# zhengjingsen/LidarDetection

Hardware: AMD Instinct MI355X
Metric: frames/sec (fwd+NMS) PointPillar-KITTI (higher is better)
Workload: dtype f32; 1 GPU; PointPillar-KITTI bs=16 per GPU, fp32, eval BN folded: HIP voxelize + PFN; dense 2D backbone = first layer from the pillars (sparse implicit GEMM), stride-1 3x3 layers as Winograd F(4x4,3x3) on the fp32 MFMA, strided deblocks as one fused MFMA GEMM (all this repo's HIP), the two stride-2 3x3 layers MIOpen, stride-1 deblock + 1x1 heads hipBLASLt; exact HIP top-k + decode + batched rotated NMS; clou; replicas=1

## Files before the change

### include/lidar_hip.h

```cpp
#ifndef LIDAR_HIP_H
#define LIDAR_HIP_H

#include <stddef.h>
#include <stdint.h>

#ifdef __cplusplus
extern "C" {
#endif

#define LIDAR_OK 0
#define LIDAR_ERR_ARG (-1)
#define LIDAR_ERR_LAUNCH (-2)
#define LIDAR_ERR_WORKSPACE (-3)
#define LIDAR_ERR_UNSUPPORTED (-4)

size_t lidar_voxelize_workspace_bytes(int batch, int n_max, int max_voxels);
int lidar_voxelize_workspace_init(void *ws, size_t ws_bytes, int batch, int n_max, int max_voxels, void *stream);
int lidar_voxelize(const float *points, const int *point_offsets, int batch, int n_max, int num_features,
                   const float *range6, const float *voxel_size3, const int *grid3, int max_points,
                   int max_voxels, int compact, int algo, float *voxels, int *coords, int *num_points,
                   int *voxel_offsets, void *ws, size_t ws_bytes, void *stream);
int lidar_voxelize_hostoff(const float *points, const int *point_offsets, const int *host_offsets, int batch, int n_max,
                           int num_features, const float *range6, const float *voxel_size3, const int *grid3, int max_points,
                           int max_voxels, int compact, int algo, float *voxels, int *coords, int *num_points,
// ... 192 lines not shown
                                             int n_out, int K, int Cin, int Cout, const float *packed, const float *bias,
                                             const float *residual, int relu, float *out_features, void *stream);
int lidar_spconv_wgrad(const float *in_features, const float *grad_out, const int *nbr, int n_out, int K, int Cin, int Cout,
                       float *grad_weight, void *stream);
int lidar_spconv_wgrad_mfma_supported(int K, int Cin, int Cout);
size_t lidar_spconv_wgrad_workspace_bytes(int n_out, int K, int Cin, int Cout);
int lidar_spconv_wgrad_mfma(const float *in_features, const float *grad_out, const int *nbr, const int *order, int n_out, int K,
                            int Cin, int Cout, float *grad_weight, void *ws, size_t ws_bytes, void *stream);
size_t lidar_sparse_to_dense_workspace_bytes(int batch, int D, int H, int W);
int lidar_sparse_to_dense(const float *features, const int *indices, int n, int channels, int batch, int D, int H, int W,
                          float *out, void *ws, size_t ws_bytes, void *stream);

int lidar_bias_act_nhwc(const float *in, const float *bias, long long n_pix, int C, int relu, float *out, int out_C,
                        int out_off, void *stream);
int lidar_bias_act_upsample_nhwc(const float *in, const float *bias, int batch, int h, int w, int s, int C, int relu,
                                 float *out, int out_C, int out_off, void *stream);
int lidar_dense_gemm_bias_act(const float *A, long long M, int K, const float *W, int N, const float *bias, int relu,
                              float *D, int ldd, void *ws, size_t ws_bytes, void *stream);
int lidar_dense_gemm_export_choices(int *out7, int cap);
int lidar_dense_gemm_import_choices(const int *in7, int n);

size_t lidar_wino_packed_floats(int Cin, int Cout);
int lidar_wino_supported(int Cin, int Cout);
int lidar_wino_pack_weights(const float *w, int Cin, int Cout, float *packed, void *stream);
int lidar_wino_conv3x3_nhwc(const float *in, int B, int H, int W, int Cin, const float *packed, const float *bias, int relu, int Cout,
                            float *out, int out_C, int out_off, void *stream);
int lidar_wino_conv3x3_grouped_nhwc(const float *in, int B, int H, int W, int in_C, int group_cin, int n_groups, const float *packed,
                                    const float *bias, int relu, float *out, int out_C, int out_off, void *stream);
int lidar_wino_conv3x3_grouped_compact_nhwc(const float *in, int B, int H, int W, int in_C, int group_cin, int n_groups,
                                            const float *packed, const float *bias, int relu, const int *grp_cout, const int *grp_ooff,
                                            float *out, int out_C, int out_off, void *stream);

size_t lidar_wino43_packed_floats(int Cin, int Cout);
int lidar_wino43_supported(int Cin, int Cout);
int lidar_wino43_pack_weights(const float *w, int Cin, int Cout, float *packed, void *stream);
int lidar_wino43_conv3x3_nhwc(const float *in, int B, int H, int W, int Cin, int in_C, const float *packed, const float *bias, int relu,
                              int Cout, float *out, int out_C, int out_off, void *stream);
size_t lidar_wino43s_packed_floats(int Cin, int Cout);
int lidar_wino43s_supported(int Cin, int Cout);
int lidar_wino43s_pack_weights(const float *w, int Cin, int Cout, float *packed, void *stream);
int lidar_wino43s_conv3x3_nhwc(const float *in, int B, int H, int W, int Cin, int in_C, const float *packed, const float *bias, int relu,
                               int Cout, float *out, int out_C, int out_off, void *stream);

int lidar_wino43_wgrad_supported(int Cin, int Cout);
size_t lidar_wino43_wgrad_workspace_bytes(int B, int H, int W, int Cin, int Cout);
int lidar_wino43_wgrad_nhwc(const float *x, int x_ld, const float *g, int g_ld, int B, int H, int W, int Cin, int Cout, float *dw,
                            void *ws, size_t ws_bytes, void *stream);

size_t lidar_deconv_packed_floats(int K, int N);
int lidar_deconv_supported(int K, int s, int C_up);
int lidar_deconv_pack_weights(const float *W, int K, int N, float *packed, void *stream);
int lidar_deconv_gemm_nhwc(const float *in, int B, int h, int w, int K, const float *packed, const float *bias, int relu, int s, int C_up,
                           float *out, int out_C, int out_off, void *stream);

#define LIDAR_DECONV_TRAIN_MIN_K 16
#define LIDAR_DECONV_TRAIN_MIN_CUP 32
#define LIDAR_DECONV_TRAIN_MAX_C 512
int lidar_deconv_train_supported(int K, int s, int C_up);
size_t lidar_deconv_wgrad_workspace_bytes(int B, int h, int w, int K, int s, int C_up);
int lidar_deconv_dgrad_nhwc(const float *g, int g_ld, const float *W, int B, int h, int w, int K, int s, int C_up, float *dx, int dx_ld,
                            void *stream);
int lidar_deconv_wgrad_nhwc(const float *x, int x_ld, const float *g, int g_ld, int B, int h, int w, int K, int s, int C_up, float *dw,
                            void *ws, size_t ws_bytes, void *stream);

int lidar_anchor_scores(const float *head, long long n_loc, int row_stride, int cls_off, int anchors_per_loc, int num_class,
                        float score_thresh, float *scores, unsigned char *labels, void *stream);
int lidar_decode_topk(const float *head, int batch, long long locs_per_frame, int row_stride, int box_off, int dir_off,
                      int anchors_per_loc, int num_dir_bins, const long long *top_idx, int k, const float *anchors,
                      float dir_offset, float dir_limit_offset, float period, float *boxes, void *stream);
size_t lidar_topk_workspace_bytes(int batch, long long n);
int lidar_topk_workspace_init(void *ws, size_t ws_bytes, int batch, long long n, void *stream);
int lidar_anchor_scores_hist(const float *head, int batch, long long locs_per_frame, int row_stride, int cls_off, int anchors_per_loc,
                             int num_class, float score_thresh, float *scores, unsigned char *labels, void *ws, size_t ws_bytes,
                             void *stream);
int lidar_topk_desc(const float *scores, int batch, long long n, int k, float valid_min, float score_max, int hist_ready,
                    float *top_scores, long long *top_idx, int *counts, void *ws, size_t ws_bytes, void *stream);
int lidar_post_nms_gather(const float *boxes, const float *top_scores, const long long *top_idx, const unsigned char *labels,
                          const long long *keep, const int *num_keep, int batch, int k, long long n, int keep_stride, int post,
                          float *out_boxes, float *out_scores, long long *out_labels, int *out_num, void *stream);

size_t lidar_anchor_assign_workspace_bytes(int batch, int max_gt, int num_classes);
int lidar_anchor_assign(const float *const *anchors, const long long *counts, const long long *per_loc, const long long *out_off,
                        const float *matched, const float *unmatched, const int *remap, int num_classes, int anchor_dim,
                        long long a_total, const signed char *class_of_id, const float *gt, const float *gt_enlarged, int batch,
                        int max_gt, int gt_cols, int code_size, int sincos, int norm_by_num_examples, int *labels, float *targets,
                        float *weights, void *ws, size_t ws_bytes, void *stream);

int lidar_atss_assign_supported(const long long *counts, int num_sets, int anchor_dim, int gt_cols, int code_size, int sincos,
                                int topk, int max_gt, int match_height);
size_t lidar_atss_assign_workspace_bytes(int batch, int max_gt, int num_sets, int topk);
int lidar_atss_assign(const float *const *anchors, const long long *counts, int num_sets, int anchor_dim, const float *gt, int batch,
                      int max_gt, int gt_cols, int code_size, int sincos, int topk, int match_height, int *labels, float *targets,
                      float *weights, void *ws, size_t ws_bytes, void *stream);

#define LIDAR_PROPOSAL_TARGET_MAX_ROIS 1024
#define LIDAR_PROPOSAL_TARGET_MAX_GT 512
#define LIDAR_PROPOSAL_TARGET_MAX_SAMPLES 512
#define LIDAR_PROPOSAL_TARGET_MAX_DIM 16
int lidar_proposal_target_supported(int num_rois, int max_gt, int roi_per_image, int box_dim);
int lidar_proposal_target(const float *rois, const float *roi_scores, const long long *roi_labels, const float *gt_boxes,
                          const float *gt_boxes_enlarged, int batch, int num_rois, int max_gt, int box_dim, int roi_per_image,
                          int fg_rois_per_image, const int *hard_quota, int by_class, int cls_score_type, float reg_fg_thresh,
                          float cls_fg_thresh, float cls_bg_thresh, float cls_bg_thresh_lo, float cls_fg_minus_bg,
                          const float *fg_keys, const float *draws, float *out_rois, float *out_gt_of_rois,
                          float *out_gt_of_rois_src, float *out_iou, float *out_scores, long long *out_labels,
                          long long *out_reg_valid, float *out_cls_labels, int *out_sampled, int *frame_status,
// ... 112 lines not shown
```

### lidardetection_amd/_lib.py

```python
import ctypes as C
import os

_HERE = os.path.dirname(os.path.abspath(__file__))
SO_PATH = os.environ.get("LIDAR_HIP_SO") or os.path.join(_HERE, "csrc", "liblidar_hip.so")

vp, i32, f32, sz = C.c_void_p, C.c_int, C.c_float, C.c_size_t

SIGNATURES = {
    "lidar_voxelize_workspace_bytes": (sz, [i32, i32, i32]),
    "lidar_voxelize_workspace_init": (i32, [vp, sz, i32, i32, i32, vp]),
    "lidar_voxelize": (i32, [vp, vp, i32, i32, i32, vp, vp, vp, i32, i32, i32, i32, vp, vp, vp, vp, vp, sz, vp]),
    "lidar_voxelize_hostoff": (i32, [vp, vp, vp, i32, i32, i32, vp, vp, vp, i32, i32, i32, i32, vp, vp, vp, vp, vp, sz, vp]),
    "lidar_voxelize_error_flag": (i32, [vp, sz, i32, i32, i32]),
    "lidar_timer_create": (vp, []),
    "lidar_timer_destroy": (None, [vp]),
    "lidar_voxelize_time_next": (None, [vp]),
    "lidar_timer_elapsed_ms": (C.c_float, [vp]),
    "lidar_timer_parts_ms": (i32, [vp, vp]),
    "lidar_voxelize_set_error_mirror": (i32, [vp, sz, i32, i32, i32, vp, vp]),
    "lidar_pillar_vfe": (i32, [vp, vp, vp, i32, vp, i32, i32, vp, vp, vp, i32, vp, vp, i32, i32, i32, vp, vp]),
    "lidar_mean_vfe": (i32, [vp, vp, i32, i32, i32, i32, vp, vp]),
    "lidar_pillar_scatter_workspace_bytes": (sz, [i32, i32, i32]),
    "lidar_pillar_scatter": (i32, [vp, vp, i32, i32, vp, i32, i32, i32, i32, i32, vp, vp, sz, vp]),
    "lidar_pillar_scatter_update": (i32, [vp, vp, i32, i32, vp, i32, i32, i32, i32, vp, vp, vp, vp]),
# ... 59 lines not shown
    "lidar_spconv_grid_init": (i32, [vp, sz, vp]),
    "lidar_spconv_grid_rows": (i32, [vp, i32, vp, i32, i32, i32, i32, vp, i32, vp]),
    "lidar_spconv_grid_table": (i32, [vp, i32, i32, i32, i32, i32, i32, i32, i32, i32, i32, i32, i32, i32, i32, vp, i32, vp, vp]),
    "lidar_spconv_grid_table_t": (i32, [vp, i32, i32, i32, i32, i32, i32, i32, i32, i32, i32, i32, i32, i32, i32, vp, i32, vp, vp]),
    "lidar_spconv_grid_pad_rows": (i32, [vp, vp, i32, vp]),
    "lidar_spconv_transpose_table": (i32, [vp, i32, i32, i32, vp, vp]),
    "lidar_spconv_grid_outputs_workspace_bytes": (sz, [i32, i32]),
    "lidar_spconv_grid_outputs": (i32, [vp, i32, i32, i32, i32, i32, i32, i32, i32, i32, i32, i32, i32, i32, i32, vp, vp, vp, vp, sz, vp]),
    "lidar_spconv_implicit_gemm": (i32, [vp, vp, i32, i32, i32, i32, vp, vp, vp, vp]),
    "lidar_spconv_implicit_gemm_fused": (i32, [vp, vp, i32, i32, i32, i32, vp, vp, vp, i32, vp, vp]),
    "lidar_spconv_row_masks": (i32, [vp, i32, i32, vp, vp]),
    "lidar_spconv_mask_group_workspace_bytes": (sz, [i32]),
    "lidar_spconv_mask_group_init": (i32, [vp, sz, vp]),
    "lidar_spconv_mask_group": (i32, [vp, i32, i32, vp, vp, vp, sz, vp]),
    "lidar_spconv_sorted_gemm_supported": (i32, [i32, i32, i32]),
    "lidar_spconv_implicit_gemm_sorted": (i32, [vp, vp, vp, vp, i32, i32, i32, i32, vp, vp, vp, i32, vp, vp]),
    "lidar_spconv_packed_floats": (sz, [i32, i32, i32]),
    "lidar_spconv_pack_weights": (i32, [vp, i32, i32, i32, vp, vp]),
    "lidar_spconv_implicit_gemm_sorted_packed": (i32, [vp, vp, vp, vp, i32, i32, i32, i32, vp, vp, vp, i32, vp, vp]),
    "lidar_spconv_wgrad": (i32, [vp, vp, vp, i32, i32, i32, i32, vp, vp]),
    "lidar_spconv_wgrad_mfma_supported": (i32, [i32, i32, i32]),
    "lidar_spconv_wgrad_workspace_bytes": (sz, [i32, i32, i32, i32]),
    "lidar_spconv_wgrad_mfma": (i32, [vp, vp, vp, vp, i32, i32, i32, i32, vp, vp, sz, vp]),
    "lidar_sparse_to_dense_workspace_bytes": (sz, [i32, i32, i32, i32]),
    "lidar_sparse_to_dense": (i32, [vp, vp, i32, i32, i32, i32, i32, i32, vp, vp, sz, vp]),
    "lidar_sparse_to_bev_nhwc": (i32, [vp, vp, i32, i32, i32, i32, i32, i32, vp, vp, sz, vp]),
    "lidar_sparse_to_bev_nhwc_backward": (i32, [vp, i32, i32, vp, i32, i32, i32, i32, i32, i32, vp, vp]),
    "lidar_bias_act_nhwc": (i32, [vp, vp, C.c_longlong, i32, i32, vp, i32, i32, vp]),
    "lidar_bias_act_upsample_nhwc": (i32, [vp, vp, i32, i32, i32, i32, i32, i32, vp, i32, i32, vp]),
    "lidar_dense_gemm_bias_act": (i32, [vp, C.c_longlong, i32, vp, i32, vp, i32, vp, i32, vp, sz, vp]),
    "lidar_dense_gemm_export_choices": (i32, [vp, i32]),
    "lidar_dense_gemm_import_choices": (i32, [vp, i32]),
    "lidar_wino_packed_floats": (sz, [i32, i32]),
    "lidar_wino_supported": (i32, [i32, i32]),
    "lidar_wino_pack_weights": (i32, [vp, i32, i32, vp, vp]),
    "lidar_wino_conv3x3_nhwc": (i32, [vp, i32, i32, i32, i32, vp, vp, i32, i32, vp, i32, i32, vp]),
    "lidar_wino43_packed_floats": (sz, [i32, i32]),
    "lidar_wino43_supported": (i32, [i32, i32]),
    "lidar_wino43_pack_weights": (i32, [vp, i32, i32, vp, vp]),
    "lidar_wino43_conv3x3_nhwc": (i32, [vp, i32, i32, i32, i32, i32, vp, vp, i32, i32, vp, i32, i32, vp]),
    "lidar_wino43s_packed_floats": (sz, [i32, i32]),
    "lidar_wino43s_supported": (i32, [i32, i32]),
    "lidar_wino43s_pack_weights": (i32, [vp, i32, i32, vp, vp]),
    "lidar_wino43s_conv3x3_nhwc": (i32, [vp, i32, i32, i32, i32, i32, vp, vp, i32, i32, vp, i32, i32, vp]),
    "lidar_wino43_wgrad_supported": (i32, [i32, i32]),
    "lidar_wino43_wgrad_workspace_bytes": (sz, [i32, i32, i32, i32, i32]),
    "lidar_wino43_wgrad_nhwc": (i32, [vp, i32, vp, i32, i32, i32, i32, i32, i32, vp, vp, sz, vp]),
    "lidar_wino_conv3x3_grouped_nhwc": (i32, [vp, i32, i32, i32, i32, i32, i32, vp, vp, i32, vp, i32, i32, vp]),
    "lidar_wino_conv3x3_grouped_compact_nhwc": (i32, [vp, i32, i32, i32, i32, i32, i32, vp, vp, i32, vp, vp, vp, i32, i32, vp]),
    "lidar_deconv_packed_floats": (sz, [i32, i32]),
    "lidar_deconv_supported": (i32, [i32, i32, i32]),
    "lidar_deconv_pack_weights": (i32, [vp, i32, i32, vp, vp]),
    "lidar_deconv_gemm_nhwc": (i32, [vp, i32, i32, i32, i32, vp, vp, i32, i32, i32, vp, i32, i32, vp]),
    "lidar_deconv_train_supported": (i32, [i32, i32, i32]),
    "lidar_deconv_wgrad_workspace_bytes": (sz, [i32, i32, i32, i32, i32, i32]),
    "lidar_deconv_dgrad_nhwc": (i32, [vp, i32, vp, i32, i32, i32, i32, i32, i32, vp, i32, vp]),
    "lidar_deconv_wgrad_nhwc": (i32, [vp, i32, vp, i32, i32, i32, i32, i32, i32, i32, vp, vp, sz, vp]),
    "lidar_anchor_scores": (i32, [vp, C.c_longlong, i32, i32, i32, i32, f32, vp, vp, vp]),
    "lidar_decode_topk": (i32, [vp, i32, C.c_longlong, i32, i32, i32, i32, i32, vp, i32, vp, f32, f32, f32, vp, vp]),
    "lidar_topk_workspace_bytes": (sz, [i32, C.c_longlong]),
    "lidar_topk_workspace_init": (i32, [vp, sz, i32, C.c_longlong, vp]),
    "lidar_anchor_scores_hist": (i32, [vp, i32, C.c_longlong, i32, i32, i32, i32, f32, vp, vp, vp, sz, vp]),
    "lidar_topk_desc": (i32, [vp, i32, C.c_longlong, i32, f32, f32, i32, vp, vp, vp, vp, sz, vp]),
    "lidar_post_nms_gather": (i32, [vp, vp, vp, vp, vp, vp, i32, i32, C.c_longlong, i32, i32, vp, vp, vp, vp, vp]),
    "lidar_anchor_assign_workspace_bytes": (sz, [i32, i32, i32]),
    "lidar_anchor_assign": (i32, [vp, vp, vp, vp, vp, vp, vp, i32, i32, C.c_longlong, vp, vp, vp, i32, i32, i32, i32, i32, i32, vp,
                                  vp, vp, vp, sz, vp]),
    "lidar_atss_assign_supported": (i32, [vp, i32, i32, i32, i32, i32, i32, i32, i32]),
    "lidar_atss_assign_workspace_bytes": (sz, [i32, i32, i32, i32]),
    "lidar_atss_assign": (i32, [vp, vp, i32, i32, vp, i32, i32, i32, i32, i32, i32, i32, vp, vp, vp, vp, sz, vp]),
    "lidar_proposal_target_supported": (i32, [i32, i32, i32, i32]),
    "lidar_proposal_target": (i32, [vp, vp, vp, vp, vp, i32, i32, i32, i32, i32, i32, vp, i32, i32, f32, f32, f32, f32, f32, vp, vp,
                                    vp, vp, vp, vp, vp, vp, vp, vp, vp, vp, vp, vp, vp]),
    "lidar_augment_supported": (i32, [i32, i32, i32, i32]),
    "lidar_augment_workspace_bytes": (sz, [i32, i32, i32, i32]),
    "lidar_augment": (i32, [vp, vp, i32, i32, vp, vp, i32, i32, vp, vp, vp, vp, i32, i32, vp, i32, i32, vp, vp, vp, vp, vp, vp, vp,
                            vp, vp, vp, i32, i32, C.c_longlong, i32, vp, vp, vp, vp, vp, vp, sz, vp]),
    "lidar_anchor_loss_workspace_bytes": (sz, [i32, vp, i32]),
    "lidar_anchor_loss_forward": (i32, [vp, vp, vp, vp, vp, vp, i32, vp, vp, vp, i32, i32, C.c_longlong, i32, i32, i32, vp, vp, i32,
                                        vp, vp, sz, vp]),
    "lidar_anchor_loss_backward": (i32, [vp, vp, vp, vp, vp, vp, i32, vp, vp, vp, i32, i32, C.c_longlong, i32, i32, i32, vp, vp, i32,
                                         vp, vp, vp, vp, vp, sz, vp]),
    "lidar_roi_loss_supported": (i32, [i32, i32, i32, i32, i32, i32]),
    "lidar_roi_loss_workspace_bytes": (sz, [i32, i32]),
    "lidar_roi_loss_forward": (i32, [vp, vp, vp, vp, vp, vp, vp, i32, i32, vp, vp, i32, vp, vp, sz, vp]),
    "lidar_roi_loss_backward": (i32, [i32, i32, vp, vp, i32, vp, vp, vp, vp, sz, vp]),
    "lidar_point_head_supported": (i32, [C.c_longlong, i32, i32, i32, i32, i32]),
    "lidar_point_targets": (i32, [vp, C.c_longlong, vp, i32, i32, i32, vp, i32, i32, vp, i32, vp, vp, vp, vp, vp]),
    "lidar_point_loss_ws_bytes": (sz, [C.c_longlong]),
    "lidar_point_loss_forward": (i32, [vp, vp, vp, vp, vp, vp, C.c_longlong, i32, vp, vp, vp, vp, sz, vp]),
    "lidar_point_loss_backward": (i32, [vp, vp, vp, vp, vp, vp, C.c_longlong, i32, vp, vp, vp, vp, vp, vp, vp, sz, vp]),
    "lidar_optim_plan": (C.c_longlong, [vp, i32, vp, vp, C.c_longlong]),
    "lidar_optim_workspace_bytes": (sz, [C.c_longlong]),
    "lidar_optim_grad_norm": (i32, [vp, i32, vp, vp, C.c_longlong, f32, vp, vp, sz, vp]),
    "lidar_optim_adam_step": (i32, [vp, i32, vp, vp, C.c_longlong, vp, C.c_double, C.c_double, C.c_double, C.c_double, C.c_double,
                                    C.c_longlong, i32, vp]),
    "lidar_rotate_iou_eval": (i32, [vp, i32, vp, i32, i32, vp, vp]),
    "lidar_kitti_eval_supported": (i32, [i32, C.c_longlong, C.c_longlong, i32, i32, i32, i32, i32]),
    "lidar_kitti_eval_workspace_bytes": (sz, [i32, C.c_longlong, C.c_longlong, i32, i32, i32, i32, i32]),
    "lidar_kitti_eval_overlaps": (i32, [i32, i32, vp, vp, vp, vp, vp, i32, C.c_longlong, C.c_longlong, C.c_longlong, i32, i32, vp, vp]),
    "lidar_kitti_eval_class": (i32, [i32, vp, vp, vp, vp, vp, vp, vp, vp, vp, i32, C.c_longlong, C.c_longlong, C.c_longlong, i32, i32,
                                     vp, i32, vp, i32, vp, i32, i32, vp, vp, vp, vp, vp, vp, vp, sz, vp]),
    "lidar_boxes_iou_bev_cpu":(i32, [vp, i32, vp, i32, vp]),
    "lidar_points_in_boxes_cpu": (i32, [vp, i32, vp, i32, vp]),
    "lidar_voxelize_cpu_scratch_bytes": (sz, [i32]),
    "lidar_voxelize_cpu": (i32, [vp, i32, i32, vp, vp, vp, i32, i32, vp, vp, vp, vp, sz]),
# ... 116 lines not shown
```

### lidardetection_amd/bev_backbone.py

```python
import ctypes as C
import os
from typing import NamedTuple, Optional

import torch
import torch.nn as nn
import torch.nn.functional as F

from . import _lib, wino, workspace


def bias_act_(x, bias, relu=True, out=None, out_offset=0):
    _lib.require_cuda(bias)
    if not (x.is_cuda and x.dim() == 4 and x.is_contiguous(memory_format=torch.channels_last)):
        raise _lib.LidarHipError("bias_act_: expected a channels-last CUDA tensor")
    B, C, H, W = x.shape
    out, out_offset = (x, 0) if out is None else _lib.nhwc_out("bias_act_", B, (H, W), C, x.device, out, out_offset)
    _lib.check(_lib.lib().lidar_bias_act_nhwc(_lib.ptr(x), _lib.ptr(bias), B * H * W, C, int(bool(relu)), _lib.ptr(out),
                                              out.shape[1], int(out_offset), _lib.stream()), "lidar_bias_act_nhwc")
    return out


_LT_GEMM = [os.environ.get("LIDAR_BEV_LT_GEMM", "1") != "0"]
_SPLIT_MIN = [int(os.environ.get("LIDAR_BEV_SPLIT_MIN", "8"))]
_SPLIT = [int(os.environ.get("LIDAR_BEV_SPLIT", "2"))]
# ... 22 lines not shown
            st = pool[dev] = torch.cuda.Stream(dev, priority=-1)
        out.append(st)
    return out


def gemm_bias_act_into_(x, w_kn, bias, out, out_offset, relu=True):
    _lib.require_cuda(w_kn, bias)
    _lib.require_nhwc(x, "gemm_bias_act_into_")
    B, K, h, w = x.shape
    N = w_kn.shape[1]
    if w_kn.shape[0] != K or bias.numel() != N:
        raise _lib.LidarHipError("gemm_bias_act_into_: shapes do not match")
    out, out_offset = _lib.nhwc_out("gemm_bias_act_into_", B, (h, w), N, x.device, out, out_offset)
    return _lt_gemm(_lib.ptr(x), B * h * w, K, w_kn, bias, relu, C.c_void_p(out.data_ptr() + 4 * out_offset), out.shape[1], x.device)


def rows_gemm(a2d, w_kn, bias=None, out=None):
    if _LT_GEMM[0] and a2d.is_cuda and a2d.dtype == torch.float32 and a2d.is_contiguous() and w_kn.is_contiguous():
        if out is None:
            out = torch.empty((a2d.shape[0], w_kn.shape[1]), dtype=torch.float32, device=a2d.device)
        elif not out.is_contiguous() or out.shape != (a2d.shape[0], w_kn.shape[1]):
            raise _lib.LidarHipError("rows_gemm: out must be a contiguous (M, N) tensor")
        if _lt_gemm(_lib.ptr(a2d), a2d.shape[0], a2d.shape[1], w_kn, bias, False, _lib.ptr(out), w_kn.shape[1], a2d.device):
            return out
        _LT_GEMM[0] = False
    if out is None:
        return torch.mm(a2d, w_kn) if bias is None else torch.addmm(bias, a2d, w_kn)
    return torch.mm(a2d, w_kn, out=out) if bias is None else torch.addmm(bias, a2d, w_kn, out=out)


def deconv_supported(K, s, c_up):
    return bool(_lib.lib().lidar_deconv_supported(int(K), int(s), int(c_up)))


def deconv_pack(w_kn):
    _lib.require_cuda(w_kn)
    K, N = w_kn.shape
    L = _lib.lib()
    n = L.lidar_deconv_packed_floats(K, N)
    if n == 0:
        raise _lib.LidarHipError(f"deconv_pack: unsupported shape ({K}, {N})")
    packed = torch.empty(n, dtype=torch.float32, device=w_kn.device)
    _lib.check(L.lidar_deconv_pack_weights(_lib.ptr(w_kn.contiguous()), K, N, _lib.ptr(packed), _lib.stream()), "lidar_deconv_pack_weights")
    return packed


_DECONV_MAX_BYTES = [2 ** 31 - 1]


def deconv_fits(B, K, h, w, s, out_c):
    return B * h * w * K * 4 < _DECONV_MAX_BYTES[0] and B * h * w * s * s * out_c * 4 < _DECONV_MAX_BYTES[0]


def deconv_gemm_into_(x, packed, bias, s, out, out_offset=0, relu=True):
    _lib.require_cuda(packed, bias)
    _lib.require_nhwc(x, "deconv_gemm_into_")
    B, K, h, w = x.shape
    c_up = bias.numel()
    if packed.numel() != K * s * s * c_up:
        raise _lib.LidarHipError("deconv_gemm_into_: packed weights do not match (K, s, C_up)")
    out, out_offset = _lib.nhwc_out("deconv_gemm_into_", B, (s * h, s * w), c_up, x.device, out, out_offset)
    _lib.check(_lib.lib().lidar_deconv_gemm_nhwc(_lib.ptr(x), B, h, w, K, _lib.ptr(packed), _lib.ptr(bias), int(bool(relu)), int(s), c_up,
                                                 _lib.ptr(out), out.shape[1], int(out_offset), _lib.stream()), "lidar_deconv_gemm_nhwc")
    return out


def bias_act_upsample_(y2d, bias, batch, h, w, s, out, out_offset=0, relu=True):
    _lib.require_cuda(y2d, bias)
    C = bias.numel()
    if y2d.shape != (batch * h * w, s * s * C):
        raise _lib.LidarHipError("bias_act_upsample_: GEMM output shape does not match (batch*h*w, s*s*C)")
    out, out_offset = _lib.nhwc_out("bias_act_upsample_", batch, (h * s, w * s), C, y2d.device, out, out_offset)
    _lib.check(_lib.lib().lidar_bias_act_upsample_nhwc(_lib.ptr(y2d), _lib.ptr(bias), batch, h, w, s, C, int(bool(relu)),
                                                       _lib.ptr(out), out.shape[1], int(out_offset), _lib.stream()),
               "lidar_bias_act_upsample_nhwc")
    return out


def collect_params(*modules):
    out = []
    for m in modules:
        out += list(m.parameters()) + list(m.buffers())
    return out


def params_key(tensors):
    return tuple((t.data_ptr(), t._version) for t in tensors)


def _fold(weight, bn, out_dim, conv_bias=None):
    scale = bn.weight.detach() / torch.sqrt(bn.running_var + bn.eps)
    shift = bn.bias.detach() - bn.running_mean * scale
    if conv_bias is not None:
        shift = shift + conv_bias.detach() * scale
    shape = [1] * weight.dim()
    shape[out_dim] = -1
    return (weight.detach() * scale.view(shape)), shift.contiguous()


class BlockLayer(NamedTuple):
    zpad: Optional[nn.ZeroPad2d]
    conv: nn.Conv2d
    bn: nn.BatchNorm2d
    act: Optional[nn.ReLU]
    pad: Optional[tuple]
    zero_pad: Optional[tuple]

    @property
    def plain3x3(self):
        c = self.conv
        return (self.pad == (1, 1) and self.zero_pad is None and tuple(c.kernel_size) == (3, 3) and tuple(c.stride) == (1, 1)
                and tuple(c.dilation) == (1, 1) and c.groups == 1)


def block_layer(zpad, conv, bn, act=None):
    pad, zero_pad = None, None if zpad is None else tuple(int(v) for v in zpad.padding)
# ... 200 lines not shown
```

### lidardetection_amd/csrc/deconv_gemm.hip

```cpp
#include "common.h"
#ifndef DC_PROBE
#define DC_PROBE 0
#endif

typedef float f32x16 __attribute__((ext_vector_type(16)));
typedef float f32x4 __attribute__((ext_vector_type(4)));
typedef unsigned u32x4 __attribute__((ext_vector_type(4)));
typedef float f32x2 __attribute__((ext_vector_type(2)));

#define DC_OOB 0x80000000u

__global__ __launch_bounds__(256) void dc_pack_kernel(const float *__restrict__ W, int K, int N, float *__restrict__ P) {
    const long long idx = (long long)blockIdx.x * 256 + threadIdx.x;
    if (idx >= (long long)K * N) return;
    const int k = (int)(idx / N), col = (int)(idx - (long long)k * N);
    const int c = k >> 2, h = (k >> 1) & 1, s = k & 1, g = col >> 9, t = (col >> 5) & 15, j = col & 31, NG = N >> 9;
    P[(((((size_t)c * NG + g) * 8 + (t >> 1)) * 64 + (h * 32 + j)) * 2 + (t & 1)) * 2 + s] = W[idx];
}

struct DcArgs {
    const float *in;
    const float *pk;
    const float *bias;
    float *out;
    int P, K, N, h, w, s, C_up, out_C, out_off, relu;
    int n_pblocks, n_groups, n_blocks;
    unsigned out_bytes;
};

#define DC_STG_PITCH 132
static constexpr size_t dc_lds_bytes() { return (size_t)2 * 128 * 16 + (size_t)4 * 32 * DC_STG_PITCH * 4; }

__global__ __launch_bounds__(256) void dc_gemm_kernel(const DcArgs a) {
    extern __shared__ float4 s_mem4[];
    float4 *s_a = s_mem4;
    float *s_stg = reinterpret_cast<float *>(s_mem4 + 2 * 128);
    const int t = threadIdx.x, l = t & 63, wv = __builtin_amdgcn_readfirstlane(t >> 6);
    const int i = l & 31, h = l >> 5;
    const int K = a.K, NC = K >> 2;
    const int bstride = a.n_groups * 8 * 64;

    const int nb8 = (a.n_blocks + 7) >> 3;
    const __amdgpu_buffer_rsrc_t orsrc = __builtin_amdgcn_make_buffer_rsrc(a.out, (short)0, (int)a.out_bytes, 0x00020000);
    const int xcd = (int)(blockIdx.x & 7), slot = (int)(blockIdx.x >> 3), nslots = (int)(gridDim.x >> 3);
    const int blk_end = min((xcd + 1) * nb8, a.n_blocks);
    int blk = xcd * nb8 + slot;
    if (blk >= blk_end) return;

    struct Tile {
        unsigned aoff;
        int b;
        int p0, g;
    };
    auto make_tile = [&](int blk_) {
        Tile tl;
        tl.g = blk_ % a.n_groups;
        const int pb = blk_ / a.n_groups;
        tl.p0 = pb * 128;
        const int p = tl.p0 + 64 * (wv & 1) + l;
        tl.aoff = p < a.P ? (unsigned)p * (unsigned)K * 4u : DC_OOB;
        tl.b = tl.g * 8 * 64;
        return tl;
    };
    typedef int i32x4 __attribute__((ext_vector_type(4)));
    i32x4 arsrc;
    {
        const unsigned long long base = (unsigned long long)a.in;
        arsrc[0] = (int)(unsigned)base;
        arsrc[1] = (int)((unsigned)(base >> 32) & 0xffffu);
        arsrc[2] = (int)((unsigned)a.P * (unsigned)K * 4u);
        arsrc[3] = 0x00020000;
    }
    const __amdgpu_buffer_rsrc_t brsrc = __builtin_amdgcn_make_buffer_rsrc(const_cast<float *>(a.pk), (short)0, (int)((unsigned)K * (unsigned)a.N * 4u), 0x00020000);
    const int l16 = l * 16;
    auto ldb = [&](int f4_index) { return __builtin_bit_cast(f32x4, __builtin_amdgcn_raw_buffer_load_b128(brsrc, l16, f4_index * 16, 0)); };
    const unsigned a_lds = (unsigned)(size_t)((__attribute__((address_space(3))) char *)s_a);
    unsigned doff = 0;
    auto dma = [&](int buf) {
        if (wv < 2) {
            const unsigned dst = a_lds + (unsigned)((buf * 128 + 64 * wv) * 16);
            asm volatile("s_mov_b32 m0, %2\n\ts_nop 0\n\tbuffer_load_dwordx4 %0, %1, 0 offen lds" : : "v"(doff), "s"(arsrc), "s"(dst) : "memory", "m0");
        }
    };
    auto load_a = [&](int buf, f32x2 &av) { av = reinterpret_cast<const f32x2 *>(s_a + buf * 128 + 32 * wv + i)[h]; };

    f32x16 acc[16];
    f32x2 a0, a1;
    f32x4 b0[8], b1[8];
    Tile cur = make_tile(blk), nxt = cur;
    doff = cur.aoff;
    dma(0);
    doff += 16u;
    dma(1);
    doff += 16u;
#pragma unroll
    for (int e = 0; e < 8; ++e) b0[e] = ldb(cur.b + e * 64);
    __builtin_amdgcn_s_waitcnt(0x0F70);
    asm volatile("" ::: "memory");
    __syncthreads();
    load_a(0, a0);
    __syncthreads();

#define DC_CHUNK(c, P, FIRST, AC, BC, AN, BN)                                                                                      \
    {                                                                                                                              \
        if ((c) > 0) {                                                                                                             \
            if (DC_PROBE & 1) asm volatile("s_waitcnt lgkmcnt(0)\n\ts_barrier" ::: "memory");                                      \
            else asm volatile("s_waitcnt vmcnt(8) lgkmcnt(0)\n\ts_barrier" ::: "memory");                                          \
        } else if (!first_block) asm volatile("s_waitcnt lgkmcnt(0)\n\ts_barrier" ::: "memory");                                   \
        dma(P);                                                                                        \
        doff = ((c) + 3 == NC) ? (has_next ? nxt.aoff : DC_OOB) : doff + 16u;                                                      \
        const int bn_ = ((c) + 1 < NC) ? cur.b + ((c) + 1) * bstride : (has_next ? nxt.b : cur.b);                                 \
        const f32x2 *as_ = reinterpret_cast<const f32x2 *>(s_a + (1 - (P)) * 128 + 32 * wv + i) + h;                               \
        __builtin_amdgcn_sched_barrier(0);                                                                                         \
        _Pragma("unroll") for (int k = 0; k < 32; ++k) {                                                                           \
            const float bop_ = BC[(k & 15) >> 1][((k & 1) << 1) + (k >> 4)];                                                       \
            if (FIRST && k < 16) {                                                                                                 \
                f32x16 z_;                                                                                                         \
                _Pragma("unroll") for (int r_ = 0; r_ < 16; ++r_) z_[r_] = 0.f;                                                    \
                acc[k & 15] = __builtin_amdgcn_mfma_f32_32x32x2f32(AC[k >> 4], bop_, z_, 0, 0, 0);                                 \
            } else {                                                                                                               \
                acc[k & 15] = __builtin_amdgcn_mfma_f32_32x32x2f32(AC[k >> 4], bop_, acc[k & 15], 0, 0, 0);                        \
            }                                                                                                                      \
            if (k < 8) BN[k] = ldb(bn_ + k * 64);                                                                                  \
            if (k == 2) AN = as_[0];                                                                                               \
            __builtin_amdgcn_sched_barrier(0);                                                                                     \
        }                                                                                                                          \
    }

    bool first_block = true;
    for (;;) {
        const int blk_next = blk + nslots;
        const bool has_next = blk_next < blk_end;
        if (has_next) nxt = make_tile(blk_next);
        DC_CHUNK(0, 0, true, a0, b0, a1, b1)
        DC_CHUNK(1, 1, false, a1, b1, a0, b0)
        for (int c = 2; c < NC; c += 2) {
            DC_CHUNK(c, 0, false, a0, b0, a1, b1)
            DC_CHUNK(c + 1, 1, false, a1, b1, a0, b0)
        }
        {
            __builtin_amdgcn_s_waitcnt(0x0F70);
            int lo = l;
            asm volatile("" : "+v"(lo));
            const bool relu = a.relu != 0;
            float *stg = s_stg + (size_t)wv * 32 * DC_STG_PITCH;
            const int hw = a.h * a.w, OW = a.s * a.w;
            unsigned pix[16];
            {
                const int p = cur.p0 + 32 * wv + (lo >> 5);
                int bb = p / hw;
                const int rem = p - bb * hw;
                int y = rem / a.w, x = rem - y * a.w;
#pragma unroll
                for (int k = 0; k < 16; ++k) {
                    pix[k] = (p + 2 * k < a.P) ? (unsigned)(((bb * a.s * a.h + a.s * y) * OW + a.s * x) * a.out_C + a.out_off + 4 * (lo & 31)) * 4u : 0x80000000u;
#pragma unroll
                    for (int st = 0; st < 2; ++st) {
                        x += 1;
                        if (x >= a.w) { x = 0; y += 1; }
                        if (y >= a.h) { y = 0; bb += 1; }
                    }
                }
            }
#pragma unroll
            for (int rnd = 0; rnd < 4; ++rnd) {
                const int col0 = 512 * cur.g + 128 * rnd;
                const int kk = col0 / a.C_up, c0 = col0 - kk * a.C_up;
                const int ky = kk / a.s, kx = kk - ky * a.s;
#pragma unroll
                for (int nn = 0; nn < 4; ++nn) {
                    const float bvv = a.bias ? a.bias[c0 + 32 * nn + i] : 0.f;
                    float m[16];
#pragma unroll
                    for (int r = 0; r < 16; ++r) asm volatile("v_accvgpr_read_b32 %0, %1" : "=v"(m[r]) : "a"(acc[4 * rnd + nn][r]));
#pragma unroll
                    for (int r = 0; r < 16; ++r) {
                        const int row = 8 * (r >> 2) + 4 * h + (r & 3);
                        const float v = m[r] + bvv;
                        stg[row * DC_STG_PITCH + 32 * nn + i] = relu ? fmaxf(v, 0.f) : v;
                    }
                    __builtin_amdgcn_sched_barrier(0);
                }
                const int soff = ((ky * OW + kx) * a.out_C + c0) * 4;
#pragma unroll
                for (int k4 = 0; k4 < 16; k4 += 4) {
                    f32x4 sv[4];
#pragma unroll
                    for (int k = 0; k < 4; ++k) sv[k] = *reinterpret_cast<const f32x4 *>(stg + (2 * (k4 + k) + (lo >> 5)) * DC_STG_PITCH + 4 * (lo & 31));
#pragma unroll
                    for (int k = 0; k < 4; ++k)
                        __builtin_amdgcn_raw_buffer_store_b128(__builtin_bit_cast(u32x4, sv[k]), orsrc, (int)pix[k4 + k], soff, 0);
                    __builtin_amdgcn_sched_barrier(0);
                }
            }
        }
        if (!has_next) break;
        cur = nxt;
        blk = blk_next;
        first_block = false;
    }
#undef DC_CHUNK
}

LIDAR_EXPORT size_t lidar_deconv_packed_floats(int K, int N) {
    if (K < 16 || N <= 0 || (K & 7) || (N & 511)) return 0;
    return (size_t)K * N;
}

LIDAR_EXPORT int lidar_deconv_supported(int K, int s, int C_up) {
    if (s <= 0 || C_up <= 0 || (C_up & 127)) return 0;
    return lidar_deconv_packed_floats(K, s * s * C_up) != 0;
}

LIDAR_EXPORT int lidar_deconv_pack_weights(const float *W, int K, int N, float *packed, void *stream) {
    if (!W || !packed || lidar_deconv_packed_floats(K, N) == 0) return LIDAR_ERR_ARG;
    hipLaunchKernelGGL(dc_pack_kernel, dim3(divup((long long)K * N, 256)), dim3(256), 0, (hipStream_t)stream, W, K, N, packed);
    return lidar_check_launch("lidar_deconv_pack_weights");
}

static int dc_cu_count() {
    static int cus[64] = {};
    int dev = 0, n = 0;
    if (hipGetDevice(&dev) != hipSuccess) return 256;
    dev &= 63;
    if (cus[dev] == 0) cus[dev] = (hipDeviceGetAttribute(&n, hipDeviceAttributeMultiprocessorCount, dev) == hipSuccess && n > 0) ? n : 256;
    return cus[dev];
}

LIDAR_EXPORT int lidar_deconv_gemm_nhwc(const float *in, int B, int h, int w, int K, const float *packed, const float *bias, int relu, int s,
                                        int C_up, float *out, int out_C, int out_off, void *stream) {
    if (!in || !packed || !out || B <= 0 || h <= 0 || w <= 0 || !lidar_deconv_supported(K, s, C_up) || out_off < 0 || out_off + C_up > out_C)
        return LIDAR_ERR_ARG;
    if ((reinterpret_cast<uintptr_t>(in) & 15) || (reinterpret_cast<uintptr_t>(packed) & 15) || (reinterpret_cast<uintptr_t>(out) & 15) ||
        (out_C & 3) || (out_off & 3) || (long long)B * h * w > 0x7fffffffll || (long long)B * h * w * s * s * out_C * 4 >= 0x7fffffffll ||
        (long long)B * h * w * K * 4 >= 0x7fffffffll || (long long)K * s * s * C_up * 4 >= 0x7fffffffll)
        return LIDAR_ERR_ARG;
    DcArgs a;
    a.in = in; a.pk = packed; a.bias = bias; a.out = out;
    a.P = B * h * w; a.K = K; a.N = s * s * C_up; a.h = h; a.w = w; a.s = s; a.C_up = C_up; a.out_C = out_C; a.out_off = out_off; a.relu = relu;
    a.out_bytes = (unsigned)((long long)B * h * w * s * s * out_C * 4);
    a.n_pblocks = divup(a.P, 128);
    a.n_groups = a.N / 512;
    const long long nblk = (long long)a.n_pblocks * a.n_groups;
    if (nblk > 0x7ffffff0ll) return LIDAR_ERR_ARG;
    a.n_blocks = (int)nblk;
    long long want = ((nblk + 7) / 8) * 8;
    const long long cap = ((long long)dc_cu_count() / 8) * 8;
    if (cap >= 8 && want > cap) want = cap;
    static bool attr_set[64] = {};
    int dev_id = 0;
    (void)hipGetDevice(&dev_id);
    dev_id &= 63;
    if (!attr_set[dev_id]) {
        (void)hipFuncSetAttribute(reinterpret_cast<const void *>(&dc_gemm_kernel), hipFuncAttributeMaxDynamicSharedMemorySize, (int)dc_lds_bytes());
        attr_set[dev_id] = true;
    }
    hipLaunchKernelGGL(dc_gemm_kernel, dim3((unsigned)want), dim3(256), dc_lds_bytes(), (hipStream_t)stream, a);
    return lidar_check_launch("lidar_deconv_gemm_nhwc");
}
```

Baseline: 3296 frames/s.

## Halve deconv GEMM wave column tile to 256 for two-wave occupancy

Templates the fused strided-deconv MFMA GEMM on the per-wave column count and makes 256 columns the default, down from 512. This halves the accumulator registers, and launch bounds allow two blocks per CU, with the persistent grid cap doubled to match. The packed weight layout is generalized to the new column grouping, and an environment variable can switch back to the 512 path. The aim is better latency hiding through occupancy, at the cost of more A-operand reloads per output column.

```diff
diff --git a/include/lidar_hip.h b/include/lidar_hip.h
--- a/include/lidar_hip.h
+++ b/include/lidar_hip.h
@@ -268,6 +268,10 @@
 int lidar_deconv_pack_weights(const float *W, int K, int N, float *packed, void *stream);
 int lidar_deconv_gemm_nhwc(const float *in, int B, int h, int w, int K, const float *packed, const float *bias, int relu, int s, int C_up,
                            float *out, int out_C, int out_off, void *stream);
+int lidar_deconv_route_cols(int K, int s, int C_up, long long P);
+long long lidar_deconv_pack_index(int K, int N, int k, int col, int cols);
+int lidar_deconv_gemm_nhwc_cols(const float *in, int B, int h, int w, int K, const float *packed, const float *bias, int relu, int s, int C_up,
+                                float *out, int out_C, int out_off, int cols, void *stream);
 
 #define LIDAR_DECONV_TRAIN_MIN_K 16
 #define LIDAR_DECONV_TRAIN_MIN_CUP 32
diff --git a/lidardetection_amd/_lib.py b/lidardetection_amd/_lib.py
--- a/lidardetection_amd/_lib.py
+++ b/lidardetection_amd/_lib.py
@@ -135,6 +135,9 @@
     "lidar_deconv_supported": (i32, [i32, i32, i32]),
     "lidar_deconv_pack_weights": (i32, [vp, i32, i32, vp, vp]),
     "lidar_deconv_gemm_nhwc": (i32, [vp, i32, i32, i32, i32, vp, vp, i32, i32, i32, vp, i32, i32, vp]),
+    "lidar_deconv_route_cols": (i32, [i32, i32, i32, C.c_longlong]),
+    "lidar_deconv_pack_index": (C.c_longlong, [i32, i32, i32, i32, i32]),
+    "lidar_deconv_gemm_nhwc_cols": (i32, [vp, i32, i32, i32, i32, vp, vp, i32, i32, i32, vp, i32, i32, i32, vp]),
     "lidar_deconv_train_supported": (i32, [i32, i32, i32]),
     "lidar_deconv_wgrad_workspace_bytes": (sz, [i32, i32, i32, i32, i32, i32]),
     "lidar_deconv_dgrad_nhwc": (i32, [vp, i32, vp, i32, i32, i32, i32, i32, i32, vp, i32, vp]),
diff --git a/lidardetection_amd/bev_backbone.py b/lidardetection_amd/bev_backbone.py
--- a/lidardetection_amd/bev_backbone.py
+++ b/lidardetection_amd/bev_backbone.py
@@ -98,7 +98,11 @@
     return B * h * w * K * 4 < _DECONV_MAX_BYTES[0] and B * h * w * s * s * out_c * 4 < _DECONV_MAX_BYTES[0]
 
 
-def deconv_gemm_into_(x, packed, bias, s, out, out_offset=0, relu=True):
+def deconv_route_cols(K, s, c_up, pixels):
+    return int(_lib.lib().lidar_deconv_route_cols(int(K), int(s), int(c_up), int(pixels)))
+
+
+def deconv_gemm_into_(x, packed, bias, s, out, out_offset=0, relu=True, cols=0):
     _lib.require_cuda(packed, bias)
     _lib.require_nhwc(x, "deconv_gemm_into_")
     B, K, h, w = x.shape
@@ -106,8 +110,9 @@
     if packed.numel() != K * s * s * c_up:
         raise _lib.LidarHipError("deconv_gemm_into_: packed weights do not match (K, s, C_up)")
     out, out_offset = _lib.nhwc_out("deconv_gemm_into_", B, (s * h, s * w), c_up, x.device, out, out_offset)
-    _lib.check(_lib.lib().lidar_deconv_gemm_nhwc(_lib.ptr(x), B, h, w, K, _lib.ptr(packed), _lib.ptr(bias), int(bool(relu)), int(s), c_up,
-                                                 _lib.ptr(out), out.shape[1], int(out_offset), _lib.stream()), "lidar_deconv_gemm_nhwc")
+    _lib.check(_lib.lib().lidar_deconv_gemm_nhwc_cols(_lib.ptr(x), B, h, w, K, _lib.ptr(packed), _lib.ptr(bias), int(bool(relu)), int(s), c_up,
+                                                      _lib.ptr(out), out.shape[1], int(out_offset), int(cols), _lib.stream()),
+               "lidar_deconv_gemm_nhwc")
     return out
 
 
diff --git a/lidardetection_amd/csrc/deconv_gemm.hip b/lidardetection_amd/csrc/deconv_gemm.hip
--- a/lidardetection_amd/csrc/deconv_gemm.hip
+++ b/lidardetection_amd/csrc/deconv_gemm.hip
@@ -1,4 +1,5 @@
 #include "common.h"
+#include <stdlib.h>
 #ifndef DC_PROBE
 #define DC_PROBE 0
 #endif
@@ -10,12 +11,17 @@
 
 #define DC_OOB 0x80000000u
 
+__host__ __device__ static inline size_t dc_pack_index(int N, int k, int col, int cols) {
+    const int T = cols >> 5, NG = N / cols;
+    const int c = k >> 2, h = (k >> 1) & 1, s = k & 1, g = col / cols, t = (col >> 5) & (T - 1), j = col & 31;
+    return (((((size_t)c * NG + g) * (T >> 1) + (t >> 1)) * 64 + (h * 32 + j)) * 2 + (t & 1)) * 2 + s;
+}
+
 __global__ __launch_bounds__(256) void dc_pack_kernel(const float *__restrict__ W, int K, int N, float *__restrict__ P) {
     const long long idx = (long long)blockIdx.x * 256 + threadIdx.x;
     if (idx >= (long long)K * N) return;
     const int k = (int)(idx / N), col = (int)(idx - (long long)k * N);
-    const int c = k >> 2, h = (k >> 1) & 1, s = k & 1, g = col >> 9, t = (col >> 5) & 15, j = col & 31, NG = N >> 9;
-    P[(((((size_t)c * NG + g) * 8 + (t >> 1)) * 64 + (h * 32 + j)) * 2 + (t & 1)) * 2 + s] = W[idx];
+    P[dc_pack_index(N, k, col, 256)] = W[idx];
 }
 
 struct DcArgs {
@@ -31,14 +37,17 @@
 #define DC_STG_PITCH 132
 static constexpr size_t dc_lds_bytes() { return (size_t)2 * 128 * 16 + (size_t)4 * 32 * DC_STG_PITCH * 4; }
 
-__global__ __launch_bounds__(256) void dc_gemm_kernel(const DcArgs a) {
+template <int COLS>
+__global__ __launch_bounds__(256, COLS == 256 ? 2 : 1) void dc_gemm_kernel(const DcArgs a) {
+    static_assert(COLS == 512 || COLS == 256, "a wave owns 512 or 256 columns");
+    constexpr int NT = COLS / 32, NB = NT / 2;
     extern __shared__ float4 s_mem4[];
     float4 *s_a = s_mem4;
     float *s_stg = reinterpret_cast<float *>(s_mem4 + 2 * 128);
     const int t = threadIdx.x, l = t & 63, wv = __builtin_amdgcn_readfirstlane(t >> 6);
     const int i = l & 31, h = l >> 5;
     const int K = a.K, NC = K >> 2;
-    const int bstride = a.n_groups * 8 * 64;
+    const int bstride = a.n_groups * NB * 64;
 
     const int nb8 = (a.n_blocks + 7) >> 3;
     const __amdgpu_buffer_rsrc_t orsrc = __builtin_amdgcn_make_buffer_rsrc(a.out, (short)0, (int)a.out_bytes, 0x00020000);
@@ -59,7 +68,7 @@
         tl.p0 = pb * 128;
         const int p = tl.p0 + 64 * (wv & 1) + l;
         tl.aoff = p < a.P ? (unsigned)p * (unsigned)K * 4u : DC_OOB;
-        tl.b = tl.g * 8 * 64;
+        tl.b = tl.g * NB * 64;
         return tl;
     };
     typedef int i32x4 __attribute__((ext_vector_type(4)));
@@ -84,9 +93,9 @@
     };
     auto load_a = [&](int buf, f32x2 &av) { av = reinterpret_cast<const f32x2 *>(s_a + buf * 128 + 32 * wv + i)[h]; };
 
-    f32x16 acc[16];
+    f32x16 acc[NT];
     f32x2 a0, a1;
-    f32x4 b0[8], b1[8];
+    f32x4 b0[NB], b1[NB];
     Tile cur = make_tile(blk), nxt = cur;
     doff = cur.aoff;
     dma(0);
@@ -94,7 +103,7 @@
     dma(1);
     doff += 16u;
 #pragma unroll
-    for (int e = 0; e < 8; ++e) b0[e] = ldb(cur.b + e * 64);
+    for (int e = 0; e < NB; ++e) b0[e] = ldb(cur.b + e * 64);
     __builtin_amdgcn_s_waitcnt(0x0F70);
     asm volatile("" ::: "memory");
     __syncthreads();
@@ -105,23 +114,24 @@
     {                                                                                                                              \
         if ((c) > 0) {                                                                                                             \
             if (DC_PROBE & 1) asm volatile("s_waitcnt lgkmcnt(0)\n\ts_barrier" ::: "memory");                                      \
-            else asm volatile("s_waitcnt vmcnt(8) lgkmcnt(0)\n\ts_barrier" ::: "memory");                                          \
+            else if (NB == 8) asm volatile("s_waitcnt vmcnt(8) lgkmcnt(0)\n\ts_barrier" ::: "memory");                             \
+            else asm volatile("s_waitcnt vmcnt(4) lgkmcnt(0)\n\ts_barrier" ::: "memory");                                          \
         } else if (!first_block) asm volatile("s_waitcnt lgkmcnt(0)\n\ts_barrier" ::: "memory");                                   \
         dma(P);                                                                                        \
         doff = ((c) + 3 == NC) ? (has_next ? nxt.aoff : DC_OOB) : doff + 16u;                                                      \
         const int bn_ = ((c) + 1 < NC) ? cur.b + ((c) + 1) * bstride : (has_next ? nxt.b : cur.b);                                 \
         const f32x2 *as_ = reinterpret_cast<const f32x2 *>(s_a + (1 - (P)) * 128 + 32 * wv + i) + h;                               \
         __builtin_amdgcn_sched_barrier(0);                                                                                         \
-        _Pragma("unroll") for (int k = 0; k < 32; ++k) {                                                                           \
-            const float bop_ = BC[(k & 15) >> 1][((k & 1) << 1) + (k >> 4)];                                                       \
-            if (FIRST && k < 16) {                                                                                                 \
+        _Pragma("unroll") for (int k = 0; k < 2 * NT; ++k) {                                                                       \
+            const float bop_ = BC[(k % NT) >> 1][((k & 1) << 1) + (k / NT)];                                                       \
+            if (FIRST && k < NT) {                                                                                                 \
                 f32x16 z_;                                                                                                         \
                 _Pragma("unroll") for (int r_ = 0; r_ < 16; ++r_) z_[r_] = 0.f;                                                    \
-                acc[k & 15] = __builtin_amdgcn_mfma_f32_32x32x2f32(AC[k >> 4], bop_, z_, 0, 0, 0);                                 \
+                acc[k % NT] = __builtin_amdgcn_mfma_f32_32x32x2f32(AC[k / NT], bop_, z_, 0, 0, 0);                                 \
             } else {                                                                                                               \
-                acc[k & 15] = __builtin_amdgcn_mfma_f32_32x32x2f32(AC[k >> 4], bop_, acc[k & 15], 0, 0, 0);                        \
+                acc[k % NT] = __builtin_amdgcn_mfma_f32_32x32x2f32(AC[k / NT], bop_, acc[k % NT], 0, 0, 0);                        \
             }                                                                                                                      \
-            if (k < 8) BN[k] = ldb(bn_ + k * 64);                                                                                  \
+            if (k < NB) BN[k] = ldb(bn_ + k * 64);                                                                                 \
             if (k == 2) AN = as_[0];                                                                                               \
             __builtin_amdgcn_sched_barrier(0);                                                                                     \
         }                                                                                                                          \
@@ -163,8 +173,8 @@
                 }
             }
 #pragma unroll
-            for (int rnd = 0; rnd < 4; ++rnd) {
-                const int col0 = 512 * cur.g + 128 * rnd;
+            for (int rnd = 0; rnd < NT / 4; ++rnd) {
+                const int col0 = COLS * cur.g + 128 * rnd;
                 const int kk = col0 / a.C_up, c0 = col0 - kk * a.C_up;
                 const int ky = kk / a.s, kx = kk - ky * a.s;
 #pragma unroll
@@ -227,9 +237,43 @@
     return cus[dev];
 }
 
-LIDAR_EXPORT int lidar_deconv_gemm_nhwc(const float *in, int B, int h, int w, int K, const float *packed, const float *bias, int relu, int s,
-                                        int C_up, float *out, int out_C, int out_off, void *stream) {
-    if (!in || !packed || !out || B <= 0 || h <= 0 || w <= 0 || !lidar_deconv_supported(K, s, C_up) || out_off < 0 || out_off + C_up > out_C)
+LIDAR_EXPORT int lidar_deconv_route_cols(int K, int s, int C_up, long long P) {
+    if (!lidar_deconv_supported(K, s, C_up) || P <= 0) return 0;
+    const char *e = getenv("LIDAR_DC_OCC2");
+    if (e && e[0] == '0' && e[1] == 0) return 512;
+    return 256;
+}
+
+LIDAR_EXPORT long long lidar_deconv_pack_index(int K, int N, int k, int col, int cols) {
+    if (lidar_deconv_packed_floats(K, N) == 0 || (cols != 256 && cols != 512) || k < 0 || k >= K || col < 0 || col >= N) return -1;
+    return (long long)dc_pack_index(N, k, col, cols);
+}
+
+template <int COLS>
+static int dc_launch(DcArgs a, hipStream_t stream) {
+    a.n_groups = a.N / COLS;
+    const long long nblk = (long long)a.n_pblocks * a.n_groups;
+    if (nblk > 0x7ffffff0ll) return LIDAR_ERR_ARG;
+    a.n_blocks = (int)nblk;
+    long long want = ((nblk + 7) / 8) * 8;
+    const long long cap = ((long long)dc_cu_count() * (512 / COLS) / 8) * 8;
+    if (cap >= 8 && want > cap) want = cap;
+    static bool attr_set[64] = {};
+    int dev_id = 0;
+    (void)hipGetDevice(&dev_id);
+    dev_id &= 63;
+    if (!attr_set[dev_id]) {
+        (void)hipFuncSetAttribute(reinterpret_cast<const void *>(&dc_gemm_kernel<COLS>), hipFuncAttributeMaxDynamicSharedMemorySize, (int)dc_lds_bytes());
+        attr_set[dev_id] = true;
+    }
+    hipLaunchKernelGGL(dc_gemm_kernel<COLS>, dim3((unsigned)want), dim3(256), dc_lds_bytes(), stream, a);
+    return lidar_check_launch("lidar_deconv_gemm_nhwc");
+}
+
+LIDAR_EXPORT int lidar_deconv_gemm_nhwc_cols(const float *in, int B, int h, int w, int K, const float *packed, const float *bias, int relu, int s,
+                                             int C_up, float *out, int out_C, int out_off, int cols, void *stream) {
+    if (!in || !packed || !out || B <= 0 || h <= 0 || w <= 0 || !lidar_deconv_supported(K, s, C_up) || out_off < 0 || out_off + C_up > out_C ||
+        (cols != 0 && cols != 256 && cols != 512))
         return LIDAR_ERR_ARG;
     if ((reinterpret_cast<uintptr_t>(in) & 15) || (reinterpret_cast<uintptr_t>(packed) & 15) || (reinterpret_cast<uintptr_t>(out) & 15) ||
         (out_C & 3) || (out_off & 3) || (long long)B * h * w > 0x7fffffffll || (long long)B * h * w * s * s * out_C * 4 >= 0x7fffffffll ||
@@ -240,21 +284,11 @@
     a.P = B * h * w; a.K = K; a.N = s * s * C_up; a.h = h; a.w = w; a.s = s; a.C_up = C_up; a.out_C = out_C; a.out_off = out_off; a.relu = relu;
     a.out_bytes = (unsigned)((long long)B * h * w * s * s * out_C * 4);
     a.n_pblocks = divup(a.P, 128);
-    a.n_groups = a.N / 512;
-    const long long nblk = (long long)a.n_pblocks * a.n_groups;
-    if (nblk > 0x7ffffff0ll) return LIDAR_ERR_ARG;
-    a.n_blocks = (int)nblk;
-    long long want = ((nblk + 7) / 8) * 8;
-    const long long cap = ((long long)dc_cu_count() / 8) * 8;
-    if (cap >= 8 && want > cap) want = cap;
-    static bool attr_set[64] = {};
-    int dev_id = 0;
-    (void)hipGetDevice(&dev_id);
-    dev_id &= 63;
-    if (!attr_set[dev_id]) {
-        (void)hipFuncSetAttribute(reinterpret_cast<const void *>(&dc_gemm_kernel), hipFuncAttributeMaxDynamicSharedMemorySize, (int)dc_lds_bytes());
-        attr_set[dev_id] = true;
-    }
-    hipLaunchKernelGGL(dc_gemm_kernel, dim3((unsigned)want), dim3(256), dc_lds_bytes(), (hipStream_t)stream, a);
-    return lidar_check_launch("lidar_deconv_gemm_nhwc");
-}
+    if (cols == 0) cols = lidar_deconv_route_cols(K, s, C_up, a.P);
+    return cols == 256 ? dc_launch<256>(a, (hipStream_t)stream) : dc_launch<512>(a, (hipStream_t)stream);
+}
+
+LIDAR_EXPORT int lidar_deconv_gemm_nhwc(const float *in, int B, int h, int w, int K, const float *packed, const float *bias, int relu, int s,
+                                        int C_up, float *out, int out_C, int out_off, void *stream) {
+    return lidar_deconv_gemm_nhwc_cols(in, B, h, w, K, packed, bias, relu, s, C_up, out, out_C, out_off, 0, stream);
+}
```

New measurement: 3317 frames/s, median of 6. No clear change (+0.7%).
